# jungmannlab/picasso

Hardware: AMD Instinct MI355X
Metric: localizations/sec (7x7 ROI, MLE) (higher is better)
Workload: dtype f32+f64; 1 GPU; 10000-frame 512x512 uint16 simulated DNA-PAINT movie per GPU, 1001675 spots per GPU, 7x7 ROI MLE (sigmaxy), identify+cut+fit+table resident in HBM; frames=10000, height=512, width=512, box=7, max_it=100, localizations_total=1001675, mle_mode=refit, refit_spots_rank0=7346, frame_ranges_in_flight=2, all_gather=none

## Files before the change

__graft_entry__.py:

```python
from __future__ import annotations

import os
import subprocess
import sys

ROOT = os.path.dirname(os.path.abspath(__file__))
if ROOT not in sys.path:
    sys.path.insert(0, ROOT)


def build() -> None:
    csrc = os.path.join(ROOT, "picasso_amd", "csrc")
    jobs = str(min(4, os.cpu_count() or 1))
    subprocess.run(["make", "-C", csrc, "-j", jobs], check=True)
    subprocess.run(["make", "-C", os.path.join(ROOT, "oracle")], check=True)
    import picasso_amd
    from picasso_amd import _lib
    lib = _lib.load()
    assert lib.pmi_version() >= 100
    print(f"built {_lib.LIB_PATH} (ABI v{lib.pmi_version()}), {len(_lib.SYMBOLS)} symbols bound")


def smoke() -> None:
    import numpy as np
    import torch

    from oracle import oracle as orc
    from picasso_amd import _lib, backend, synth

    assert torch.cuda.is_available(), "smoke() needs a GPU"
    torch.cuda.set_device(0)
    _lib.require_gpu()
    cam = {"Baseline": 100.0, "Sensitivity": 1.0, "Gain": 1.0}
    movie = synth.simulate_movie(16, 256, 256, emitters_per_frame=40, seed=7, device="cuda:0")
    torch.cuda.synchronize()
    table = backend.localize_mle_device(movie.data_ptr(), np.uint16, tuple(movie.shape), 7, 5000, cam)
    host = movie.cpu().numpy()
    fr, y, x, ng = orc.identify(host, 5000, 7, threads=4)
    spots = orc.get_spots(host, fr, y, x, 7, cam)
    th, cr, ll, it = orc.gaussmle(spots, 1e-3, 100, "sigmaxy", threads=4)
    n = len(fr)
    assert n > 100 and len(table["frame"]) == n, (n, len(table["frame"]))
    assert np.array_equal(table["frame"], fr.astype(np.uint32))
    assert np.array_equal(table["net_gradient"], ng)
    assert np.array_equal(table["iterations"], it.astype(np.uint32)), int((table["iterations"] != it).sum())
    assert np.abs(table["x"] - (th[:, 0] + x - 3)).max() < 1e-3
    assert np.abs(table["y"] - (th[:, 1] + y - 3)).max() < 1e-3
# ... 11 lines not shown
```

picasso_amd/csrc/fit_common.h:

```cpp
#pragma once
#include <math.h>

#include "pmi_common.h"

namespace pmi {

#ifndef FIT_WAVES_N
#define FIT_WAVES_N 4
#endif
constexpr int FIT_WAVES = FIT_WAVES_N;
constexpr int FIT_NT = FIT_WAVES * PMI_WAVE;
constexpr int FIT_MAXPIX = PMI_MAX_BOX * PMI_MAX_BOX;

struct ConstDiv { float g, r; int fast; };
inline ConstDiv make_const_div(float g)
{
    ConstDiv c;
    c.g = g;
    c.r = (float)(1.0 / (double)g);
    c.fast = (g == g) && fabsf(g) > 1e-15f && fabsf(g) < 1e15f;
    if (g == 1.0f) c.fast = 2;
    return c;
}
__device__ __forceinline__ float div_const(float x, const ConstDiv &c)
// ... 27 lines not shown
#pragma unroll
        for (int i = 0; i < B; i++) v[i] = v[i] / c.g;
    }
}

struct FitParams {
    const float *spots;
    float *spots_out;
    const void *movie;
    const int32_t *frame, *y, *x;
    int dtype;
    int64_t Y, X;
    float baseline, sensitivity, gain;
    ConstDiv gdiv;
    int64_t N;
    const int64_t *d_n;
    int box;
    int libm_glibc;
    double eps;
    int max_it;
    float *thetas, *crlbs, *loglik;
    int32_t *iterations;
    unsigned long long *queue;
    unsigned *strict_queue;
    int64_t first;
    double *fisher;
    float eps_lo, eps_hi;
    int32_t *flag_list;
    unsigned *flag_count;
    unsigned *flag_reasons;
    const int32_t *final_list;
    const unsigned *final_list_n;
    unsigned char *refit_mark;
    float *ng_io;
    unsigned char *accept;
    int crop_y0, crop_x0, crop_cy, crop_cx;
    double min_ng;
    const int32_t *alist;
    const unsigned *alist_n;
    int32_t *alist_out;
    unsigned *alist_blk_out;
};
enum : unsigned { FLAG_MARGIN = 1u, FLAG_CURVATURE = 2u, FLAG_NARROW = 4u, FLAG_SWING = 8u, FLAG_WILD = 16u, FLAG_SLOW = 32u, FLAG_UNSTABLE = 64u };
constexpr int FLAG_REASONS = 7;
constexpr double FIT_UNSTABLE_LMAX = 1.9;
constexpr int FISHER_STRIDE = 21;
enum { FIT_STAGE_NEWTON = 1, FIT_STAGE_FINAL = 2, FIT_STAGE_INIT_ONLY = 4, FIT_STAGE_ITERATE_ONLY = 8 };
constexpr int FIT_SLOW_ITERATIONS = 64;
#ifndef PMI_MARGIN_GROWTH
#define PMI_MARGIN_GROWTH 0.0625f
#endif
constexpr float FIT_MARGIN_GROWTH = PMI_MARGIN_GROWTH;
constexpr float FIT_NARROW_SIGMA = 0.5f;
constexpr float FIT_WOBBLE_RATIO = 0.9f;
constexpr float FIT_WOBBLE_FLOOR = 1.9073486e-6f;
constexpr int FIT_WOBBLE_RUN = 3;
constexpr int FIT_WOBBLE_LATE = 9;
constexpr float FIT_TOP_FLAG = 16.0f;

template <int CTRL, int ROW_MASK = 0xf>
__device__ __forceinline__ float dpp_f(float v)
{
    return __builtin_bit_cast(float, __builtin_amdgcn_update_dpp(0, __builtin_bit_cast(int, v), CTRL, ROW_MASK, 0xf, false));
}
__device__ __forceinline__ float wave_sum(float v)
{
    v += dpp_f<0xB1>(v);
    v += dpp_f<0x4E>(v);
    v += dpp_f<0x141>(v);
    v += dpp_f<0x140>(v);
    v += dpp_f<0x142, 0xA>(v);
    v += dpp_f<0x143, 0xC>(v);
    return __builtin_bit_cast(float, __builtin_amdgcn_readlane(__builtin_bit_cast(int, v), 63));
}
template <int CTRL, int ROW_MASK = 0xf>
// ... 73 lines not shown
```

picasso_amd/csrc/gaussmle.hip:

```cpp
#include <algorithm>
#include <cmath>
#include <cstdlib>
#include <cstring>
#include <vector>

#include "fit_common.h"

namespace pmi {

__device__ __forceinline__ unsigned borderline(float D, int kk, float eps_lo, float eps_hi)
{
    const float wide = fmaxf(1.0f, (float)(kk - 1) * FIT_MARGIN_GROWTH);
    const float epsf = 0.5f * (eps_lo + eps_hi), epsm = 0.5f * (eps_hi - eps_lo) * wide;
    return ((D >= epsf - epsm && D < epsf + epsm) ? FLAG_MARGIN : 0u) | (kk > FIT_SLOW_ITERATIONS ? FLAG_SLOW : 0u);
}
struct StepHistory { float prev, prev2, wprev; int run; };
__device__ __forceinline__ bool wobbles(float st, float value, int kk, StepHistory &h)
{
    const float w = kk >= 3 ? (st - 2.0f * h.prev) + h.prev2 : 0.0f;
    const bool wob = w * h.wprev < 0.0f && fabsf(w) > FIT_WOBBLE_RATIO * fabsf(h.wprev) && fabsf(w) > FIT_WOBBLE_FLOOR * fabsf(value);
    h.run = wob ? h.run + 1 : 0;
    h.wprev = w; h.prev2 = h.prev; h.prev = st;
    return h.run >= FIT_WOBBLE_RUN || (h.run >= 2 && kk >= FIT_WOBBLE_LATE);
}
// ... 271 lines not shown
    for (int i = 0; i < NP; i++) for (int j = 0; j < NP; j++) V[i * NP + j] = (i == j) ? 1.0 : 0.0;
    for (int sweep = 0; sweep < 60; sweep++) {
        double off = 0.0;
        for (int a = 0; a < NP; a++) for (int b = a + 1; b < NP; b++) off += A[a * NP + b] * A[a * NP + b];
        if (off == 0.0) break;
        for (int a = 0; a < NP; a++)
            for (int b = a + 1; b < NP; b++) {
                double apq = A[a * NP + b];
                if (apq == 0.0) continue;
                double tau = (A[b * NP + b] - A[a * NP + a]) / (2.0 * apq);
                double tt = (tau >= 0 ? 1.0 : -1.0) / (fabs(tau) + sqrt(1.0 + tau * tau));
                double c = 1.0 / sqrt(1.0 + tt * tt), s = tt * c;
                for (int k = 0; k < NP; k++) { double x = A[k * NP + a], y = A[k * NP + b]; A[k * NP + a] = c * x - s * y; A[k * NP + b] = s * x + c * y; }
                for (int k = 0; k < NP; k++) { double x = A[a * NP + k], y = A[b * NP + k]; A[a * NP + k] = c * x - s * y; A[b * NP + k] = s * x + c * y; }
                for (int k = 0; k < NP; k++) { double x = V[k * NP + a], y = V[k * NP + b]; V[k * NP + a] = c * x - s * y; V[k * NP + b] = s * x + c * y; }
            }
    }
    double smax = 0.0;
    for (int i = 0; i < NP; i++) smax = fmax(smax, fabs(A[i * NP + i]));
    const double cutoff = 1e-15 * smax;
    for (int i = 0; i < NP; i++) {
        double acc = 0.0;
        for (int k = 0; k < NP; k++) { double lam = A[k * NP + k]; if (fabs(lam) > cutoff) acc += V[i * NP + k] * V[i * NP + k] / lam; }
        diag[i] = acc;
    }
}

template <int NP>
__global__ __launch_bounds__(256) void crlb_kernel(const double *__restrict__ fisher, int64_t first, int64_t N,
                                                   const int64_t *__restrict__ d_n, float *__restrict__ crlbs,
                                                   const int32_t *__restrict__ list, const unsigned *__restrict__ list_n,
                                                   int32_t *__restrict__ unstable, unsigned *__restrict__ unstable_n,
                                                   unsigned *__restrict__ reasons, const unsigned char *__restrict__ refit_mark,
                                                   const unsigned char *__restrict__ accept)
{
    int64_t n = N;
    if (d_n) { int64_t dn = *d_n; n = dn < n ? dn : n; }
    int64_t t = (int64_t)blockIdx.x * blockDim.x + threadIdx.x;
    int64_t sidx = first + t;
    if (list) {
        if (t >= (int64_t)*list_n) return;
        sidx = (int64_t)list[t];
        t = sidx - first;
    } else if (sidx >= n) return;
    else if (accept && !accept[sidx]) return;
    const double *f = fisher + t * FISHER_STRIDE;
    double M[36];
    {
        int e = 0;
#pragma unroll
        for (int k = 0; k < NP; k++)
#pragma unroll
            for (int l = k; l < NP; l++) { const double v = f[e++]; M[k * NP + l] = v; M[l * NP + k] = v; }
    }
    if (unstable && !(refit_mark && refit_mark[t])) {
        double dinv[NP], v[NP], lam = 0.0;
        bool ok = true;
#pragma unroll
        for (int i = 0; i < NP; i++) { const double m = M[i * NP + i]; ok = ok && m > 0.0 && m < 1e300; dinv[i] = 1.0 / sqrt(m); v[i] = 1.0 + 0.125 * (double)i; }
        if (ok) {
            double C[NP * NP], C2[NP * NP], t8 = 0.0;
#pragma unroll
            for (int i = 0; i < NP; i++)
#pragma unroll
                for (int k = 0; k < NP; k++) C[i * NP + k] = M[i * NP + k] * dinv[i] * dinv[k];
#pragma unroll
            for (int i = 0; i < NP; i++)
#pragma unroll
                for (int k = i; k < NP; k++) {
                    double a = 0.0;
#pragma unroll
                    for (int q = 0; q < NP; q++) a += C[i * NP + q] * C[q * NP + k];
                    C2[i * NP + k] = a; C2[k * NP + i] = a;
                }
#pragma unroll
            for (int i = 0; i < NP; i++)
#pragma unroll
                for (int k = i; k < NP; k++) {
// ... 239 lines not shown
    int32_t *acc_list = unstable_list + per_batch;
    unsigned *acc_blk = reinterpret_cast<unsigned *>(acc_list + per_batch);
    unsigned char *refit_mark = reinterpret_cast<unsigned char *>(acc_blk + acc_blocks);
    unsigned long long *queues = (unsigned long long *)ptr;
    unsigned *flag_counts = (unsigned *)(queues + 3 * nb);
    unsigned *strict_queues = flag_counts + 2 * nb;
    void *sptr = nullptr;
    if ((rc = scratch(SCR_STATS, 64, &sptr)) != PMI_OK) return rc;
    unsigned *stats = (unsigned *)sptr;
    hipLaunchKernelGGL(zero_words_kernel, dim3(1), dim3(256), 0, s, (unsigned *)ptr, (int)(nb * 10), stats, 16);
    p.flag_reasons = stats + 1;
    p.fisher = (double *)fptr;
    const int libm = mle_libm_now();
    const bool libm_all = libm != PMI_LIBM_DEVICE;
    p.libm_glibc = libm == PMI_LIBM_GLIBC || (libm == PMI_LIBM_AUTO && p.box <= 5);
    static const char *menv = tuning_env("PMI_MLE_MARGIN");
    const double margin = menv ? atof(menv) : g_mle_margin;
    const double ulp = ldexp(1.0, (int)floor(log2(std::max(1.0, p.box / 2.0))) - 23);
    const double margin_abs = std::max(p.eps * margin, 4.0 * ulp);
    p.eps_lo = (float)(p.eps - margin_abs);
    p.eps_hi = (float)(p.eps + margin_abs);
    const int ppl = (p.box * p.box + 63) / 64;
    const int64_t Ntotal = p.N;
    ScopedKernelTimer tm(s, &g_last_times.fit_ms);
    static const bool force_wave_per_spot = tuning_env("PMI_FIT_WAVE_PER_SPOT") != nullptr;
    const bool g8 = !force_wave_per_spot && p.box <= 15;
    float *cut = nullptr;
    static const bool no_keep = tuning_env("PMI_MLE_NO_KEEP") != nullptr;
    if (g8 && from_movie && mode != PMI_MLE_STRICT && !no_keep) {
        void *cptr = nullptr;
        if ((rc = scratch(SCR_STAGE_C, per_batch * (size_t)(p.box * p.box) * sizeof(float), &cptr)) != PMI_OK) return rc;
        cut = (float *)cptr;
    }
    p.spots_out = nullptr;
    if (p.ng_io && !(g8 && from_movie && cut)) { set_error("deferred exact stage outside the row-per-lane fit"); return PMI_ERR_ARG; }
    for (int64_t bi = 0; bi < nb; bi++) {
        p.first = bi * BATCH;
        p.N = std::min<int64_t>(Ntotal, p.first + BATCH);
        p.flag_list = mode == PMI_MLE_REFIT ? flag_list : nullptr;
        p.flag_count = flag_counts + bi;
        p.strict_queue = strict_queues + bi;
        p.refit_mark = mode == PMI_MLE_REFIT ? refit_mark : nullptr;
        if (p.refit_mark && !g8) PMI_HIP(hipMemsetAsync(refit_mark, 0, (size_t)(p.N - p.first), s));
        const int64_t count = p.N - p.first;
        const int64_t blocks = std::min<int64_t>((count + FIT_WAVES - 1) / FIT_WAVES, (int64_t)g_cu_count * 8);
        const dim3 grid((unsigned)std::max<int64_t>(blocks, 1));
        auto wave_per_spot = [&](int stages) {
            p.queue = queues + 3 * bi + (stages == FIT_STAGE_FINAL ? (p.final_list ? 2 : 1) : 0);
            if (method == PMI_MLE_SIGMAXY) {
                if (from_movie) launch_fit_ppl<6, true>(ppl, grid, s, p, stages); else launch_fit_ppl<6, false>(ppl, grid, s, p, stages);
            } else {
                if (from_movie) launch_fit_ppl<5, true>(ppl, grid, s, p, stages); else launch_fit_ppl<5, false>(ppl, grid, s, p, stages);
            }
        };
        if (mode != PMI_MLE_STRICT && g8 && from_movie && cut) {
            FitParams pi = p;
            pi.spots_out = cut;
            launch_fit_g8(pi, method, true, g_cu_count, state, FIT_STAGE_INIT_ONLY, s);
            PMI_HIP(hipGetLastError());
            FitParams q = p;
            q.spots = cut - p.first * (int64_t)(p.box * p.box);
            if (p.ng_io) {
                int32_t *al = nb == 1 && p.alist_out ? p.alist_out : acc_list;
                unsigned *ab = nb == 1 && p.alist_out ? p.alist_blk_out : acc_blk;
                if ((rc = build_accept_list(p.accept, p.first, p.N, p.d_n, ab, al, s)) != PMI_OK) return rc;
                q.alist = al;
                q.alist_n = ab + (count + ACC_BLOCK - 1) / ACC_BLOCK;
            }
            launch_fit_g8(q, method, false, g_cu_count, state, FIT_STAGE_ITERATE_ONLY, s);
            PMI_HIP(hipGetLastError());
            if (mode == PMI_MLE_REFIT)
                launch_fit_strict(q, method, false, flag_list, q.flag_count, count, g_cu_count, s);
            PMI_HIP(hipGetLastError());
            launch_fit_g8(q, method, false, g_cu_count, state, FIT_STAGE_FINAL, s);
        } else {
        if (mode == PMI_MLE_STRICT) {
            FitParams ps = p;
            ps.libm_glibc = libm_all;
            launch_fit_strict(ps, method, from_movie, nullptr, nullptr, count, g_cu_count, s);
        } else {
            if (g8) launch_fit_g8(p, method, from_movie, g_cu_count, state, FIT_STAGE_NEWTON, s);
            else wave_per_spot(FIT_STAGE_NEWTON);
            PMI_HIP(hipGetLastError());
            if (mode == PMI_MLE_REFIT)
                launch_fit_strict(p, method, from_movie, flag_list, p.flag_count, count, g_cu_count, s);
        }
        PMI_HIP(hipGetLastError());
        if (g8) launch_fit_g8(p, method, from_movie, g_cu_count, state, FIT_STAGE_FINAL, s);
        else wave_per_spot(FIT_STAGE_FINAL);
        }
        PMI_HIP(hipGetLastError());
        const unsigned cb = (unsigned)((count + 255) / 256);
        unsigned *unstable_n = flag_counts + nb + bi;
        auto crlb = [&](const int32_t *list, const unsigned *list_n, int32_t *out, unsigned *out_n) {
            if (method == PMI_MLE_SIGMAXY)
                hipLaunchKernelGGL((crlb_kernel<6>), dim3(cb), dim3(256), 0, s, p.fisher, p.first, p.N, p.d_n, p.crlbs, list, list_n, out, out_n, p.flag_reasons, p.refit_mark, p.accept);
            else
                hipLaunchKernelGGL((crlb_kernel<5>), dim3(cb), dim3(256), 0, s, p.fisher, p.first, p.N, p.d_n, p.crlbs, list, list_n, out, out_n, p.flag_reasons, p.refit_mark, p.accept);
        };
        const bool second = mode == PMI_MLE_REFIT;
        crlb(nullptr, nullptr, second ? unstable_list : nullptr, second ? unstable_n : nullptr);
        PMI_HIP(hipGetLastError());
        if (second) {
            FitParams r = p;
            r.strict_queue = strict_queues + nb + bi;
            if (cut) { r.spots = cut - p.first * (int64_t)(p.box * p.box); }
            const bool r_movie = cut ? false : from_movie;
            launch_fit_strict(r, method, r_movie, unstable_list, unstable_n, count, g_cu_count, s);
            PMI_HIP(hipGetLastError());
            r.final_list = unstable_list; r.final_list_n = unstable_n;
            if (g8) launch_fit_g8(r, method, r_movie, g_cu_count, state, FIT_STAGE_FINAL, s);
            else {
                FitParams keep = p;
                p = r;
                wave_per_spot(FIT_STAGE_FINAL);
                p = keep;
            }
            PMI_HIP(hipGetLastError());
            crlb(unstable_list, unstable_n, nullptr, nullptr);
            PMI_HIP(hipGetLastError());
        }
    }
    hipLaunchKernelGGL(flag_stats_kernel, dim3(1), dim3(1), 0, s, flag_counts, mode == PMI_MLE_REFIT ? 2 * nb : 0, stats);
    PMI_HIP(hipGetLastError());
    if ((rc = g_mle_stats.record(0, range, stats, s)) != PMI_OK) return rc;
    tm.stop();
    return PMI_OK;
}

static int read_last_stats(unsigned (&h)[16], hipStream_t s)
{
    if (g_mle_stats.valid()) PMI_HIP(hipStreamSynchronize(s));
    return g_mle_stats.read(h);
}

__global__ void cut_spots_kernel(const void *__restrict__ movie, int dtype, int64_t Y, int64_t X,
                                 const int32_t *__restrict__ frame, const int32_t *__restrict__ y,
                                 const int32_t *__restrict__ x, int64_t N, const int64_t *__restrict__ d_n,
                                 int box, float baseline, float sensitivity, ConstDiv gdiv, float *__restrict__ spots)
{
    int64_t n = N;
    if (d_n) { int64_t dn = *d_n; n = dn < n ? dn : n; }
    const int npix = box * box, h = box / 2;
    int64_t total = n * npix;
    for (int64_t t = (int64_t)blockIdx.x * blockDim.x + threadIdx.x; t < total; t += (int64_t)gridDim.x * blockDim.x) {
        int64_t i = t / npix;
        int q = (int)(t - i * npix);
        int a = q / box, c = q - a * box;
        float raw = load_movie_px(movie, dtype, ((int64_t)frame[i] * Y + (y[i] - h + a)) * X + (x[i] - h + c));
        spots[t] = div_const((raw - baseline) * sensitivity, gdiv);
    }
}
// ... 315 lines not shown
```

picasso_amd/csrc/gaussmle_g8.hip:

```cpp
#include <algorithm>

#include "fit_common.h"
#include "ng_common.h"

namespace pmi {

__device__ __forceinline__ float sum8(float v)
{
    v += dpp_f<0xB1>(v);
    v += dpp_f<0x4E>(v);
    v += dpp_f<0x141>(v);
    return v;
}
__device__ __forceinline__ float min8(float v)
{
    v = fminf(v, dpp_f<0xB1>(v));
    v = fminf(v, dpp_f<0x4E>(v));
    v = fminf(v, dpp_f<0x141>(v));
    return v;
}
__device__ __forceinline__ double sum8_d(double v)
{
    v += dpp_d<0xB1>(v);
    v += dpp_d<0x4E>(v);
// ... 516 lines not shown
    photons = (photons != photons) ? photons : (photons > 1.0 ? photons : 1.0);
    double a_sdy = 0.0, a_sy = 0.0, a_sdx = 0.0, a_sx = 0.0;
    if (rowok) {
        const float vm = d[H] - bg0;
        a_sdy = (double)vm * (double)((j - H) * (j - H));
        a_sy = (double)vm;
        if (j == H) {
#pragma unroll
            for (int i = 0; i < B; i++) {
                const float v2 = d[i] - bg0;
                a_sdx += (double)v2 * (double)((i - H) * (i - H));
                a_sx += (double)v2;
            }
        }
    }
    a_sdy = gsum_d<GS>(a_sdy); a_sy = gsum_d<GS>(a_sy); a_sdx = gsum_d<GS>(a_sdx); a_sx = gsum_d<GS>(a_sx);
    double isy = sqrt(a_sdy / a_sy), isx = sqrt(a_sdx / a_sx);
    if (!isfinite(isy)) isy = 0.01;
    if (!isfinite(isx)) isx = 0.01;
    if (isx == 0) isx = 0.01;
    if (isy == 0) isy = 0.01;

    float th[6], ms[6];
    th[0] = (float)com_x; th[1] = (float)com_y; th[2] = (float)photons; th[3] = bg0;
    if (NP == 6) { th[4] = (float)isx; th[5] = (float)isy; }
    else { th[4] = (float)((isx + isy) / 2); th[5] = 0.f; }
    ms[0] = th[4]; ms[1] = th[4];
    ms[2] = (float)(0.1 * (double)th[2]); ms[3] = (float)(0.1 * (double)th[3]);
    ms[4] = (float)(0.2 * (double)th[4]); ms[5] = (float)(0.2 * (double)th[5]);
    if (spot_ok && j == 0) {
        if (p.refit_mark) p.refit_mark[sidx - p.first] = 0;
        float4 *so = reinterpret_cast<float4 *>(state + (sidx - p.first) * 12);
        so[0] = make_float4(th[0], th[1], th[2], th[3]);
        so[1] = make_float4(th[4], th[5], ms[0], ms[1]);
        so[2] = make_float4(ms[2], ms[3], ms[4], ms[5]);
    }
}

template <int NP, int B, bool FROM_MOVIE>
__global__ __launch_bounds__(FIT_NT) void g8_iterate_kernel(FitParams p, const float *__restrict__ state)
{
    constexpr int GS = GroupOf<B>::GS, NSPW = 64 / GS;
    constexpr int REFILL_K = GS == 8 ? G8_REFILL_K : 1;
    __shared__ __attribute__((aligned(16))) float s_x[FIT_WAVES][NSPW][GLds<GS>::N];
    const int lane = threadIdx.x & 63, wid = threadIdx.x >> 6;
    const int g = lane / GS, j = lane & (GS - 1);
    const bool rowok = j < B;
    int64_t n = p.N;
    if (p.d_n) { int64_t dn = *p.d_n; n = dn < n ? dn : n; }
    const int64_t count = p.alist ? (int64_t)*p.alist_n : n - p.first;
    if (count <= 0) return;
    const int64_t total_waves = (int64_t)gridDim.x * FIT_WAVES;
    const int64_t chunk = (count + total_waves - 1) / total_waves;
    const int64_t wv = (int64_t)blockIdx.x * FIT_WAVES + __builtin_amdgcn_readfirstlane(wid);
    const int64_t base = p.alist ? 0 : p.first, lim = base + count;
    int64_t next = base + wv * chunk;
    const int64_t end = next + chunk < lim ? next + chunk : lim;
    if (next >= end) return;

    float *xs = &s_x[wid][g][0];
    float d[B], th[6], ms[6];
#pragma unroll
    for (int i = 0; i < B; i++) d[i] = 1.f;
#pragma unroll
    for (int l = 0; l < 6; l++) { th[l] = 1.f; ms[l] = 1.f; }
    LaneRole role = make_role<NP, B>(th, ms, j);
    int kk = 0;
    int64_t sidx = -1;
    bool active = false;
    unsigned flags = 0u;
    const unsigned long long below = (1ull << (lane & ~(GS - 1))) - 1ull;

    for (;;) {
        const unsigned long long pend = __ballot(!active && sidx >= 0 && j == 0);
        const unsigned long long empty = __ballot(!active && sidx < 0 && j == 0);
        const bool any_active = __any(active);
        if (__popcll(pend) >= REFILL_K || (pend != 0 && !any_active) || (empty != 0 && next < end)) {
            const unsigned gflag = gor_u<GS>(flags);
            if (!active && sidx >= 0 && j == 0) {
                float *to = p.thetas + sidx * 6;
#pragma unroll
                for (int l = 0; l < 5; l++) to[l] = th[l];
                to[5] = NP == 6 ? th[5] : th[4];
                p.iterations[sidx] = kk;
                if (gflag && p.flag_list) {
                    p.flag_list[atomicAdd(p.flag_count, 1u)] = (int32_t)sidx;
                    count_flag_reasons(p.flag_reasons, gflag);
                }
            }
            const unsigned long long want = pend | empty;
            const int64_t cand = next + __popcll(want & below);
            if (!active) {
                sidx = -1;
                if (cand < end) {
                    sidx = p.alist ? (int64_t)p.alist[cand] : cand;
                    const float4 *si = reinterpret_cast<const float4 *>(state + (sidx - p.first) * 12);
                    const float4 s0 = si[0], s1 = si[1], s2 = si[2];
                    th[0] = s0.x; th[1] = s0.y; th[2] = s0.z; th[3] = s0.w; th[4] = s1.x; th[5] = s1.y;
                    ms[0] = s1.z; ms[1] = s1.w; ms[2] = s2.x; ms[3] = s2.y; ms[4] = s2.z; ms[5] = s2.w;
                    load_row<B, FROM_MOVIE>(p, sidx, j, rowok, d);
                    role = make_role<NP, B>(th, ms, j);
                    kk = 0;
                    flags = 0u;
                    active = p.max_it > 0;
                    if (!active && j == 0) {
                        float *to = p.thetas + sidx * 6;
#pragma unroll
                        for (int l = 0; l < 5; l++) to[l] = th[l];
                        to[5] = NP == 6 ? th[5] : th[4];
                        p.iterations[sidx] = 0;
                        sidx = -1;
                    }
                }
            }
            next += __popcll(want);
            if (!__any(active)) {
                if (next >= end) break;
                continue;
            }
        } else if (!any_active) {
            break;
        }
        active = newton_step<NP, B>(d, th, role, xs, j, rowok, active, kk, p.eps, p.max_it, p.eps_lo, p.eps_hi, flags);
    }
}

template <int NP, int B, bool FROM_MOVIE>
__global__ __launch_bounds__(FIT_NT) void g8_final_kernel(FitParams p)
{
    constexpr int GS = GroupOf<B>::GS, NSPW = 64 / GS;
    __shared__ __attribute__((aligned(16))) double s_x[FIT_WAVES][NSPW][GS * 7];
    const int lane = threadIdx.x & 63, wid = threadIdx.x >> 6;
    const int g = lane / GS, j = lane & (GS - 1);
    const bool rowok = j < B;
    const float jf = (float)j;
    int64_t n = p.N;
    if (p.d_n) { int64_t dn = *p.d_n; n = dn < n ? dn : n; }
    int64_t sidx = p.first + ((int64_t)blockIdx.x * FIT_WAVES + wid) * NSPW + g;
    bool spot_ok = sidx < n;
    if (p.final_list) {
        const int64_t w0 = ((int64_t)blockIdx.x * FIT_WAVES + wid) * NSPW, items = (int64_t)*p.final_list_n;
        if (__builtin_amdgcn_readfirstlane((int)(w0 >= items))) return;
        spot_ok = w0 + g < items;
        sidx = spot_ok ? (int64_t)p.final_list[w0 + g] : p.first;
    } else if (__builtin_amdgcn_readfirstlane((int)(p.first + ((int64_t)blockIdx.x * FIT_WAVES + wid) * NSPW >= n))) return;
    else if (p.accept) spot_ok = spot_ok && p.accept[sidx] != 0;

    float d[B], th[6];
    load_row<B, FROM_MOVIE>(p, sidx, j, spot_ok && rowok, d);
#pragma unroll
    for (int l = 0; l < 6; l++) th[l] = spot_ok ? p.thetas[sidx * 6 + l] : 1.f;
    double *red = &s_x[wid][g][0];
    float *cols = reinterpret_cast<float *>(red);
    const float sgy = NP == 6 ? th[5] : th[4];
    const BTerms tx = boundary_terms(jf, th[0], th[4]);
    const BTerms ty = boundary_terms(jf, th[1], sgy);
    {
        float4 *c = reinterpret_cast<float4 *>(cols + j * 12);
        c[0] = make_float4(tx.A * tx.A, tx.A * tx.E, tx.A, tx.A * tx.S);
        c[1] = make_float4(tx.E * tx.E, tx.E, tx.E * tx.S, 1.0f);
        c[2] = make_float4(tx.S, tx.S * tx.S, 0.f, 0.f);
    }
    __builtin_amdgcn_wave_barrier();
    __threadfence_block();
    double T[10];
#pragma unroll
    for (int e = 0; e < 10; e++) T[e] = 0.0;
    float ll_loc = 0.f;
    const float N_ = th[2];
    const float NEy = N_ * ty.E;
#pragma unroll
    for (int i = 0; i < B; i++) {
        const float4 *c = reinterpret_cast<const float4 *>(cols + i * 12);
        const float4 c0 = c[0], c1 = c[1];
        const float2 c2 = *reinterpret_cast<const float2 *>(cols + i * 12 + 8);
        const float model = NEy * c1.y + th[3];
        if (rowok) {
            const double md = (double)model;
            double inv = (double)rcp_f32(model);
// ... 45 lines not shown
                const int e = j + GS * t - r0;
                if (e >= 0 && e < 7) {
                    double acc = 0.0;
#pragma unroll
                    for (int r = 0; r < B; r++) acc += red[r * 7 + e];
                    mine[t] = acc;
                }
            }
            __builtin_amdgcn_wave_barrier();
        }
    }
    double *fo = p.fisher + (sidx - p.first) * FISHER_STRIDE;
    if (spot_ok) {
#pragma unroll
        for (int t = 0; t < 3; t++)
            if (j + GS * t < NE_) fo[j + GS * t] = mine[t];
    }
    const float ll = gsum<GS>(ll_loc);
    if (spot_ok && j == 0) p.loglik[sidx] = ll;
}

template <int NP, int B, bool FROM_MOVIE>
static void launch_g8(const FitParams &p, float *state, int cu_count, int stages, hipStream_t s)
{
    constexpr int NSPW = 64 / GroupOf<B>::GS;
    const int64_t count = p.N - p.first;
    const int64_t waves = (count + NSPW - 1) / NSPW;
    const dim3 flat((unsigned)((waves + FIT_WAVES - 1) / FIT_WAVES));
    const int64_t pw = std::max<int64_t>(1, std::min<int64_t>((int64_t)cu_count * 24, (count + 63) / 64));
    const dim3 pers((unsigned)((pw + FIT_WAVES - 1) / FIT_WAVES));
    if (stages & (FIT_STAGE_NEWTON | FIT_STAGE_INIT_ONLY))
        hipLaunchKernelGGL((g8_init_kernel<NP, B, FROM_MOVIE>), flat, dim3(FIT_NT), 0, s, p, state);
    if (stages & (FIT_STAGE_NEWTON | FIT_STAGE_ITERATE_ONLY))
        hipLaunchKernelGGL((g8_iterate_kernel<NP, B, FROM_MOVIE>), pers, dim3(FIT_NT), 0, s, p, (const float *)state);
    if (stages & FIT_STAGE_FINAL)
        hipLaunchKernelGGL((g8_final_kernel<NP, B, FROM_MOVIE>), flat, dim3(FIT_NT), 0, s, p);
}

template <int NP, bool FROM_MOVIE>
static void launch_g8_box(const FitParams &p, float *state, int cu_count, int stages, hipStream_t s)
{
    switch (p.box) {
    case 3: launch_g8<NP, 3, FROM_MOVIE>(p, state, cu_count, stages, s); break;
    case 5: launch_g8<NP, 5, FROM_MOVIE>(p, state, cu_count, stages, s); break;
    case 7: launch_g8<NP, 7, FROM_MOVIE>(p, state, cu_count, stages, s); break;
    case 9: launch_g8<NP, 9, FROM_MOVIE>(p, state, cu_count, stages, s); break;
    case 11: launch_g8<NP, 11, FROM_MOVIE>(p, state, cu_count, stages, s); break;
    case 13: launch_g8<NP, 13, FROM_MOVIE>(p, state, cu_count, stages, s); break;
    default: launch_g8<NP, 15, FROM_MOVIE>(p, state, cu_count, stages, s); break;
    }
}

bool launch_fit_g8(const FitParams &p, int method, bool from_movie, int cu_count, float *state, int stages, hipStream_t s)
{
    if (p.box > 15) return false;
    if (method == PMI_MLE_SIGMAXY) {
        if (from_movie) launch_g8_box<6, true>(p, state, cu_count, stages, s); else launch_g8_box<6, false>(p, state, cu_count, stages, s);
    } else {
        if (from_movie) launch_g8_box<5, true>(p, state, cu_count, stages, s); else launch_g8_box<5, false>(p, state, cu_count, stages, s);
    }
    return true;
}

}
```

picasso_amd/csrc/pmi_common.h:

```cpp
#pragma once
#include <hip/hip_runtime.h>
#include <stdint.h>
#include <stdio.h>
#include <stdlib.h>
#include <string.h>

#include <functional>

#include "../../include/picasso_hip.h"

#define PMI_WAVE 64

namespace pmi {

#ifdef PMI_TUNING
inline const char *tuning_env(const char *name) { return getenv(name); }
#else
inline const char *tuning_env(const char *) { return nullptr; }
#endif

void set_error(const char *fmt, ...);
int hip_fail(hipError_t e, const char *what, const char *file, int line);

#define PMI_HIP(call)                                                          \
// ... 2 lines not shown
        if (e_ != hipSuccess) return pmi::hip_fail(e_, #call, __FILE__, __LINE__); \
    } while (0)

constexpr int PMI_MAX_DEVICES = 16;
int current_device();
int checked_device(int *device);
int device_cu_count();

enum ScratchSlot {
    SCR_RECORDS = 0,
    SCR_RECORDS2,
    SCR_FRAME_COUNT,
    SCR_COUNTERS,
    SCR_IDS,
    SCR_FIT,
    SCR_STAGE_A,
    SCR_STAGE_B,
    SCR_STAGE_C,
    SCR_STAGE_D,
    SCR_ROWS,
    SCR_NARROW,
    SCR_GATES,
    SCR_STATS,
    SCR_LQ_STATS,
    SCR_NUM
};
int scratch(int slot, size_t bytes, void **ptr);
int scratch_release_all();
int scratch_enter_inner();
void scratch_leave_inner(int was);
unsigned scratch_generation(int slot);
unsigned scratch_generation_of(int device, int user_bank, int slot);
int scratch_user_bank();
struct SideLane { hipStream_t s2 = nullptr; hipEvent_t ev_start = nullptr, ev_scan_a = nullptr, ev_b = nullptr, stats_done[2] = {nullptr, nullptr}; };
int side_lane(int pipeline, SideLane **lane);

struct LastFitStats {
    int device = 0, bank = 0, slot = 0;
    unsigned generation = 0;
    const unsigned *buf[2] = {nullptr, nullptr};
    hipEvent_t done[2] = {nullptr, nullptr};
    int record(int pipeline, int range, const unsigned *stats, hipStream_t s);
    bool valid() const;
    int read(unsigned (&h)[16]) const;
};

struct FusedRanges {
    size_t ids_bytes;
    int64_t capc;
    int64_t cap;
    bool rejects;
    std::function<int(void *ids, int64_t f_lo, int64_t f_hi, int64_t *d_cnt, hipStream_t st)> scan;
    std::function<int(void *ids, const int64_t *d_rows, int range, hipStream_t st)> fit;
    std::function<const unsigned *(void *ids)> accepted;
    std::function<int(void *ids, const int64_t *d_rows, const int64_t *d_row0, hipStream_t st)> table;
};
int fused_ranges(const FusedRanges &c, int pipeline, int64_t F, int64_t Y, int64_t X, int64_t f_lo, int64_t f_hi,
                 int64_t *d_out_n, hipStream_t s);

struct Record {
    int32_t frame;
    uint32_t yx;
    int32_t pad;
    float ng;
};
__host__ __device__ __forceinline__ uint32_t pack_yx(int y, int x) { return ((uint32_t)y << 16) | (uint32_t)(x & 0xffff); }
constexpr uint32_t NG_DEFERRED_BITS = 0x7fc0d1feu;
// ... 33 lines not shown
```

picasso_amd/csrc/runtime.hip:

```cpp
#include <stdarg.h>

#include <mutex>

#include "pmi_common.h"

namespace pmi {

static thread_local char g_err[512] = "";
bool g_kernel_timing = false;
KernelTimes g_last_times = {0.f, 0.f};
int g_localize_ranges = 2;
thread_local char g_last_scan_kernel[128] = "";

void set_error(const char *fmt, ...)
{
    va_list ap;
    va_start(ap, fmt);
    vsnprintf(g_err, sizeof(g_err), fmt, ap);
    va_end(ap);
}

int hip_fail(hipError_t e, const char *what, const char *file, int line)
{
    set_error("HIP error %d (%s) in %s at %s:%d", (int)e, hipGetErrorString(e), what, file, line);
// ... 77 lines not shown
        for (auto &bank : g_scratch_banks[dev])
            for (auto &b : bank)
                if (b.p) { if (hipFree(b.p) != hipSuccess) rc = PMI_ERR_HIP; b.p = nullptr; b.bytes = 0; }
    }
    (void)hipSetDevice(was);
    return rc;
}
int scratch_select_bank(int bank)
{
    if (bank < 0 || bank >= SCR_USER_BANKS) { set_error("scratch bank %d out of range", bank); return PMI_ERR_ARG; }
    g_scratch_bank = bank;
    return PMI_OK;
}
int scratch_enter_inner() { const int was = g_scratch_bank; g_scratch_bank = was % SCR_USER_BANKS + SCR_USER_BANKS; return was; }
void scratch_leave_inner(int was) { g_scratch_bank = was; }

static SideLane g_side_lanes[PMI_MAX_DEVICES][SCR_USER_BANKS][2];
static std::mutex g_side_mu;
int side_lane(int pipeline, SideLane **lane)
{
    int dev = 0;
    const int rc = checked_device(&dev);
    if (rc != PMI_OK) return rc;
    std::lock_guard<std::mutex> lk(g_side_mu);
    SideLane &sd = g_side_lanes[dev][scratch_user_bank()][pipeline ? 1 : 0];
    if (!sd.s2) {
        hipStream_t s2 = nullptr;
        PMI_HIP(hipStreamCreateWithFlags(&s2, hipStreamNonBlocking));
        PMI_HIP(hipEventCreateWithFlags(&sd.ev_start, hipEventDisableTiming));
        PMI_HIP(hipEventCreateWithFlags(&sd.ev_scan_a, hipEventDisableTiming));
        PMI_HIP(hipEventCreateWithFlags(&sd.ev_b, hipEventDisableTiming));
        PMI_HIP(hipEventCreateWithFlags(&sd.stats_done[0], hipEventDisableTiming));
        PMI_HIP(hipEventCreateWithFlags(&sd.stats_done[1], hipEventDisableTiming));
        sd.s2 = s2;
    }
    *lane = &sd;
    return PMI_OK;
}

int LastFitStats::record(int pipeline, int range, const unsigned *stats, hipStream_t s)
{
    SideLane *lane = nullptr;
    const int rc = side_lane(pipeline, &lane);
    if (rc != PMI_OK) return rc;
    PMI_HIP(hipEventRecord(lane->stats_done[range], s));
    if (range == 0) buf[1] = nullptr;
    buf[range] = stats;
    done[range] = lane->stats_done[range];
    slot = pipeline ? SCR_LQ_STATS : SCR_STATS;
    device = current_device();
    bank = scratch_user_bank();
    generation = scratch_generation_of(device, bank, slot);
    return PMI_OK;
}
bool LastFitStats::valid() const { return buf[0] && generation == scratch_generation_of(device, bank, slot); }
int LastFitStats::read(unsigned (&h)[16]) const
{
    for (unsigned &v : h) v = 0;
    if (!valid()) return PMI_OK;
    for (int k = 0; k < 2; k++) {
        if (!buf[k]) continue;
        unsigned part[16];
        PMI_HIP(hipEventSynchronize(done[k]));
        PMI_HIP(hipMemcpy(part, buf[k], 64, hipMemcpyDeviceToHost));
        for (int i = 0; i < 16; i++) h[i] += part[i];
    }
// ... 25 lines not shown
    const int64_t lo = f_lo < 0 ? 0 : f_lo, hi = f_hi > F - 1 ? F - 1 : f_hi, nf = hi - lo + 1;
    const bool two = g_localize_ranges == 2 && !g_kernel_timing && nf >= 16 && (double)nf * (double)Y * (double)X >= 2.5e8;
    void *ptr = nullptr, *cptr = nullptr;
    int rc;
    if ((rc = scratch(SCR_ROWS, 8 * sizeof(int64_t), &cptr)) != PMI_OK) return rc;
    int64_t *n = (int64_t *)cptr, *rows = n + 2;
    if ((rc = scratch(SCR_IDS, c.ids_bytes, &ptr)) != PMI_OK) return rc;
    void *ids[2] = {ptr, nullptr};
    auto table_rows = [&](hipStream_t st) {
        hipLaunchKernelGGL(table_rows_kernel, dim3(1), dim3(1), 0, st, (const int64_t *)n, c.rejects ? c.accepted(ids[0]) : nullptr,
                           (const int64_t *)(two ? n + 1 : nullptr), c.rejects && two ? c.accepted(ids[1]) : nullptr, c.capc,
                           c.cap, rows, d_out_n);
    };
    auto fit_rows = [&](int r, hipStream_t st) -> const int64_t * {
        if (!c.rejects && r == (two ? 1 : 0)) {
            table_rows(st);
            return rows + 2 + r;
        }
        hipLaunchKernelGGL(fit_rows_kernel, dim3(1), dim3(1), 0, st, (const int64_t *)(n + r), c.capc, rows + r);
        return rows + r;
    };
    if (!two) {
        if ((rc = c.scan(ids[0], f_lo, f_hi, n, s)) != PMI_OK) return rc;
        if ((rc = c.fit(ids[0], fit_rows(0, s), 0, s)) != PMI_OK) return rc;
    } else {
        SideLane *side_p = nullptr;
        if ((rc = side_lane(pipeline, &side_p)) != PMI_OK) return rc;
        SideLane &side = *side_p;
        const int64_t mid = lo + nf / 2 - 1;
        PMI_HIP(hipEventRecord(side.ev_start, s));
        PMI_HIP(hipStreamWaitEvent(side.s2, side.ev_start, 0));
        struct Join {
            SideLane &sd; hipStream_t st; bool done = false;
            ~Join() { if (!done) { (void)hipEventRecord(sd.ev_b, sd.s2); (void)hipStreamWaitEvent(st, sd.ev_b, 0); } }
        } join{side, s};
        if ((rc = c.scan(ids[0], lo, mid, n, s)) != PMI_OK) return rc;
        const int64_t *rows_a = fit_rows(0, s);
        PMI_HIP(hipEventRecord(side.ev_scan_a, s));
        if ((rc = c.fit(ids[0], rows_a, 0, s)) != PMI_OK) return rc;
        PMI_HIP(hipStreamWaitEvent(side.s2, side.ev_scan_a, 0));
        const int outer = scratch_enter_inner();
        rc = scratch(SCR_IDS, c.ids_bytes, &ids[1]);
        if (rc == PMI_OK) rc = c.scan(ids[1], mid + 1, hi, n + 1, side.s2);
        if (rc == PMI_OK) rc = c.fit(ids[1], fit_rows(1, side.s2), 1, side.s2);
        scratch_leave_inner(outer);
        if (rc != PMI_OK) return rc;
        PMI_HIP(hipEventRecord(side.ev_b, side.s2));
        PMI_HIP(hipStreamWaitEvent(s, side.ev_b, 0));
        join.done = true;
    }
    if (c.rejects) table_rows(s);
    if ((rc = c.table(ids[0], rows + 2, nullptr, s)) != PMI_OK) return rc;
    if (two && (rc = c.table(ids[1], rows + 3, rows + 4, s)) != PMI_OK) return rc;
    PMI_HIP(hipGetLastError());
    return PMI_OK;
}

void release_fft_plans();

}

extern "C" {

int pmi_version(void) { return 110; }

const char *pmi_last_error(void) { return pmi::g_err; }

// ... 90 lines not shown
```

Baseline: 368.0 million localizations/s.

## Fork MLE final/CRLB tail onto side stream, overlapping with strict refit

In refit mode the iterate kernel now writes its flag bits into an unused slot of the per-spot state. The final-stage and CRLB kernels for unflagged spots then run on a dedicated tail stream, skipping any spot marked in the state. Meanwhile the main stream runs the strict refit, then final and CRLB for only the flagged list, and the two streams join with events. The point is to overlap the long-tail strict refit with the bulk tail work, at the cost of extra streams, events and a repurposed state slot (ms[1] is now read back as ms[0]).

```diff
diff --git a/__graft_entry__.py b/__graft_entry__.py
--- a/__graft_entry__.py
+++ b/__graft_entry__.py
@@ -13,6 +13,7 @@
     csrc = os.path.join(ROOT, "picasso_amd", "csrc")
     jobs = str(min(4, os.cpu_count() or 1))
     subprocess.run(["make", "-C", csrc, "-j", jobs], check=True)
+    subprocess.run(["make", "-C", csrc, "-j", jobs, "tuning"], check=True)
     subprocess.run(["make", "-C", os.path.join(ROOT, "oracle")], check=True)
     import picasso_amd
     from picasso_amd import _lib
diff --git a/picasso_amd/csrc/fit_common.h b/picasso_amd/csrc/fit_common.h
--- a/picasso_amd/csrc/fit_common.h
+++ b/picasso_amd/csrc/fit_common.h
@@ -83,6 +83,7 @@
     const int32_t *final_list;
     const unsigned *final_list_n;
     unsigned char *refit_mark;
+    const float *skip_marked;
     float *ng_io;
     unsigned char *accept;
     int crop_y0, crop_x0, crop_cy, crop_cx;
@@ -92,6 +93,11 @@
     int32_t *alist_out;
     unsigned *alist_blk_out;
 };
+constexpr unsigned FIT_STATE_MARK = 7u;
+__device__ __forceinline__ unsigned newton_mark(const float *state, int64_t t)
+{
+    return reinterpret_cast<const unsigned *>(state)[(unsigned)t * 12u + FIT_STATE_MARK];
+}
 enum : unsigned { FLAG_MARGIN = 1u, FLAG_CURVATURE = 2u, FLAG_NARROW = 4u, FLAG_SWING = 8u, FLAG_WILD = 16u, FLAG_SLOW = 32u, FLAG_UNSTABLE = 64u };
 constexpr int FLAG_REASONS = 7;
 constexpr double FIT_UNSTABLE_LMAX = 1.9;
diff --git a/picasso_amd/csrc/gaussmle.hip b/picasso_amd/csrc/gaussmle.hip
--- a/picasso_amd/csrc/gaussmle.hip
+++ b/picasso_amd/csrc/gaussmle.hip
@@ -327,7 +327,7 @@
                                                    const int32_t *__restrict__ list, const unsigned *__restrict__ list_n,
                                                    int32_t *__restrict__ unstable, unsigned *__restrict__ unstable_n,
                                                    unsigned *__restrict__ reasons, const unsigned char *__restrict__ refit_mark,
-                                                   const unsigned char *__restrict__ accept)
+                                                   const unsigned char *__restrict__ accept, const float *__restrict__ skip_marked)
 {
     int64_t n = N;
     if (d_n) { int64_t dn = *d_n; n = dn < n ? dn : n; }
@@ -339,6 +339,7 @@
         t = sidx - first;
     } else if (sidx >= n) return;
     else if (accept && !accept[sidx]) return;
+    else if (skip_marked && newton_mark(skip_marked, t)) return;
     const double *f = fisher + t * FISHER_STRIDE;
     double M[36];
     {
@@ -644,6 +645,16 @@
         if ((rc = scratch(SCR_STAGE_C, per_batch * (size_t)(p.box * p.box) * sizeof(float), &cptr)) != PMI_OK) return rc;
         cut = (float *)cptr;
     }
+    static const bool tail_serial = tuning_env("PMI_MLE_TAIL_SERIAL") != nullptr;
+    const bool fork = mode == PMI_MLE_REFIT && g8 && !tail_serial;
+    SideLane *lane = nullptr;
+    if (fork && (rc = side_lane(0, &lane)) != PMI_OK) return rc;
+    const hipStream_t ts = fork ? lane->tail[range] : nullptr;
+    struct TailJoin {
+        SideLane *sd; const int r; const hipStream_t ts, st; bool open = false;
+        int join() { open = false; PMI_HIP(hipEventRecord(sd->ev_tail[r], ts)); PMI_HIP(hipStreamWaitEvent(st, sd->ev_tail[r], 0)); return PMI_OK; }
+        ~TailJoin() { if (open) (void)join(); }
+    } tail{lane, range, ts, s};
     p.spots_out = nullptr;
     if (p.ng_io && !(g8 && from_movie && cut)) { set_error("deferred exact stage outside the row-per-lane fit"); return PMI_ERR_ARG; }
     for (int64_t bi = 0; bi < nb; bi++) {
@@ -665,53 +676,64 @@
                 if (from_movie) launch_fit_ppl<5, true>(ppl, grid, s, p, stages); else launch_fit_ppl<5, false>(ppl, grid, s, p, stages);
             }
         };
+        FitParams f = p;
+        bool f_movie = from_movie;
         if (mode != PMI_MLE_STRICT && g8 && from_movie && cut) {
             FitParams pi = p;
             pi.spots_out = cut;
             launch_fit_g8(pi, method, true, g_cu_count, state, FIT_STAGE_INIT_ONLY, s);
             PMI_HIP(hipGetLastError());
-            FitParams q = p;
-            q.spots = cut - p.first * (int64_t)(p.box * p.box);
+            f.spots = cut - p.first * (int64_t)(p.box * p.box);
+            f_movie = false;
             if (p.ng_io) {
                 int32_t *al = nb == 1 && p.alist_out ? p.alist_out : acc_list;
                 unsigned *ab = nb == 1 && p.alist_out ? p.alist_blk_out : acc_blk;
                 if ((rc = build_accept_list(p.accept, p.first, p.N, p.d_n, ab, al, s)) != PMI_OK) return rc;
-                q.alist = al;
-                q.alist_n = ab + (count + ACC_BLOCK - 1) / ACC_BLOCK;
-            }
-            launch_fit_g8(q, method, false, g_cu_count, state, FIT_STAGE_ITERATE_ONLY, s);
-            PMI_HIP(hipGetLastError());
-            if (mode == PMI_MLE_REFIT)
-                launch_fit_strict(q, method, false, flag_list, q.flag_count, count, g_cu_count, s);
-            PMI_HIP(hipGetLastError());
-            launch_fit_g8(q, method, false, g_cu_count, state, FIT_STAGE_FINAL, s);
-        } else {
-        if (mode == PMI_MLE_STRICT) {
+                f.alist = al;
+                f.alist_n = ab + (count + ACC_BLOCK - 1) / ACC_BLOCK;
+            }
+            launch_fit_g8(f, method, false, g_cu_count, state, FIT_STAGE_ITERATE_ONLY, s);
+        } else if (mode == PMI_MLE_STRICT) {
             FitParams ps = p;
             ps.libm_glibc = libm_all;
             launch_fit_strict(ps, method, from_movie, nullptr, nullptr, count, g_cu_count, s);
         } else {
             if (g8) launch_fit_g8(p, method, from_movie, g_cu_count, state, FIT_STAGE_NEWTON, s);
             else wave_per_spot(FIT_STAGE_NEWTON);
-            PMI_HIP(hipGetLastError());
-            if (mode == PMI_MLE_REFIT)
-                launch_fit_strict(p, method, from_movie, flag_list, p.flag_count, count, g_cu_count, s);
-        }
-        PMI_HIP(hipGetLastError());
-        if (g8) launch_fit_g8(p, method, from_movie, g_cu_count, state, FIT_STAGE_FINAL, s);
-        else wave_per_spot(FIT_STAGE_FINAL);
         }
         PMI_HIP(hipGetLastError());
         const unsigned cb = (unsigned)((count + 255) / 256);
         unsigned *unstable_n = flag_counts + nb + bi;
-        auto crlb = [&](const int32_t *list, const unsigned *list_n, int32_t *out, unsigned *out_n) {
+        auto crlb = [&](hipStream_t st, const int32_t *list, const unsigned *list_n, int32_t *out, unsigned *out_n, const unsigned char *mark, const float *skip) {
             if (method == PMI_MLE_SIGMAXY)
-                hipLaunchKernelGGL((crlb_kernel<6>), dim3(cb), dim3(256), 0, s, p.fisher, p.first, p.N, p.d_n, p.crlbs, list, list_n, out, out_n, p.flag_reasons, p.refit_mark, p.accept);
+                hipLaunchKernelGGL((crlb_kernel<6>), dim3(cb), dim3(256), 0, st, p.fisher, p.first, p.N, p.d_n, p.crlbs, list, list_n, out, out_n, p.flag_reasons, mark, p.accept, skip);
             else
-                hipLaunchKernelGGL((crlb_kernel<5>), dim3(cb), dim3(256), 0, s, p.fisher, p.first, p.N, p.d_n, p.crlbs, list, list_n, out, out_n, p.flag_reasons, p.refit_mark, p.accept);
+                hipLaunchKernelGGL((crlb_kernel<5>), dim3(cb), dim3(256), 0, st, p.fisher, p.first, p.N, p.d_n, p.crlbs, list, list_n, out, out_n, p.flag_reasons, mark, p.accept, skip);
         };
         const bool second = mode == PMI_MLE_REFIT;
-        crlb(nullptr, nullptr, second ? unstable_list : nullptr, second ? unstable_n : nullptr);
+        if (fork) {
+            PMI_HIP(hipEventRecord(lane->ev_fork[range], s));
+            PMI_HIP(hipStreamWaitEvent(ts, lane->ev_fork[range], 0));
+            tail.open = true;
+            FitParams t = f;
+            t.skip_marked = state;
+            launch_fit_g8(t, method, f_movie, g_cu_count, state, FIT_STAGE_FINAL, ts);
+            crlb(ts, nullptr, nullptr, unstable_list, unstable_n, nullptr, state);
+            launch_fit_strict(f, method, f_movie, flag_list, f.flag_count, count, g_cu_count, s);
+            FitParams l = f;
+            l.final_list = flag_list; l.final_list_n = f.flag_count;
+            launch_fit_g8(l, method, f_movie, g_cu_count, state, FIT_STAGE_FINAL, s);
+            crlb(s, flag_list, f.flag_count, nullptr, nullptr, nullptr, nullptr);
+            PMI_HIP(hipGetLastError());
+            if ((rc = tail.join()) != PMI_OK) return rc;
+        } else {
+            if (mode == PMI_MLE_REFIT) launch_fit_strict(f, method, f_movie, flag_list, f.flag_count, count, g_cu_count, s);
+            PMI_HIP(hipGetLastError());
+            if (g8) launch_fit_g8(f, method, f_movie, g_cu_count, state, FIT_STAGE_FINAL, s);
+            else wave_per_spot(FIT_STAGE_FINAL);
+            PMI_HIP(hipGetLastError());
+            crlb(s, nullptr, nullptr, second ? unstable_list : nullptr, second ? unstable_n : nullptr, p.refit_mark, nullptr);
+        }
         PMI_HIP(hipGetLastError());
         if (second) {
             FitParams r = p;
@@ -729,7 +751,7 @@
                 p = keep;
             }
             PMI_HIP(hipGetLastError());
-            crlb(unstable_list, unstable_n, nullptr, nullptr);
+            crlb(s, unstable_list, unstable_n, nullptr, nullptr, nullptr, nullptr);
             PMI_HIP(hipGetLastError());
         }
     }
diff --git a/picasso_amd/csrc/gaussmle_g8.hip b/picasso_amd/csrc/gaussmle_g8.hip
--- a/picasso_amd/csrc/gaussmle_g8.hip
+++ b/picasso_amd/csrc/gaussmle_g8.hip
@@ -572,13 +572,13 @@
         if (p.refit_mark) p.refit_mark[sidx - p.first] = 0;
         float4 *so = reinterpret_cast<float4 *>(state + (sidx - p.first) * 12);
         so[0] = make_float4(th[0], th[1], th[2], th[3]);
-        so[1] = make_float4(th[4], th[5], ms[0], ms[1]);
+        so[1] = make_float4(th[4], th[5], ms[0], 0.f);
         so[2] = make_float4(ms[2], ms[3], ms[4], ms[5]);
     }
 }
 
 template <int NP, int B, bool FROM_MOVIE>
-__global__ __launch_bounds__(FIT_NT) void g8_iterate_kernel(FitParams p, const float *__restrict__ state)
+__global__ __launch_bounds__(FIT_NT) void g8_iterate_kernel(FitParams p, float *state)
 {
     constexpr int GS = GroupOf<B>::GS, NSPW = 64 / GS;
     constexpr int REFILL_K = GS == 8 ? G8_REFILL_K : 1;
@@ -624,6 +624,7 @@
                 to[5] = NP == 6 ? th[5] : th[4];
                 p.iterations[sidx] = kk;
                 if (gflag && p.flag_list) {
+                    reinterpret_cast<unsigned *>(state)[(unsigned)(sidx - p.first) * 12u + FIT_STATE_MARK] = gflag;
                     p.flag_list[atomicAdd(p.flag_count, 1u)] = (int32_t)sidx;
                     count_flag_reasons(p.flag_reasons, gflag);
                 }
@@ -637,7 +638,7 @@
                     const float4 *si = reinterpret_cast<const float4 *>(state + (sidx - p.first) * 12);
                     const float4 s0 = si[0], s1 = si[1], s2 = si[2];
                     th[0] = s0.x; th[1] = s0.y; th[2] = s0.z; th[3] = s0.w; th[4] = s1.x; th[5] = s1.y;
-                    ms[0] = s1.z; ms[1] = s1.w; ms[2] = s2.x; ms[3] = s2.y; ms[4] = s2.z; ms[5] = s2.w;
+                    ms[0] = s1.z; ms[1] = s1.z; ms[2] = s2.x; ms[3] = s2.y; ms[4] = s2.z; ms[5] = s2.w;
                     load_row<B, FROM_MOVIE>(p, sidx, j, rowok, d);
                     role = make_role<NP, B>(th, ms, j);
                     kk = 0;
@@ -684,7 +685,10 @@
         spot_ok = w0 + g < items;
         sidx = spot_ok ? (int64_t)p.final_list[w0 + g] : p.first;
     } else if (__builtin_amdgcn_readfirstlane((int)(p.first + ((int64_t)blockIdx.x * FIT_WAVES + wid) * NSPW >= n))) return;
-    else if (p.accept) spot_ok = spot_ok && p.accept[sidx] != 0;
+    else {
+        if (p.accept) spot_ok = spot_ok && p.accept[sidx] != 0;
+        if (p.skip_marked && spot_ok) spot_ok = newton_mark(p.skip_marked, sidx - p.first) == 0u;
+    }
 
     float d[B], th[6];
     load_row<B, FROM_MOVIE>(p, sidx, j, spot_ok && rowok, d);
@@ -796,7 +800,7 @@
     if (stages & (FIT_STAGE_NEWTON | FIT_STAGE_INIT_ONLY))
         hipLaunchKernelGGL((g8_init_kernel<NP, B, FROM_MOVIE>), flat, dim3(FIT_NT), 0, s, p, state);
     if (stages & (FIT_STAGE_NEWTON | FIT_STAGE_ITERATE_ONLY))
-        hipLaunchKernelGGL((g8_iterate_kernel<NP, B, FROM_MOVIE>), pers, dim3(FIT_NT), 0, s, p, (const float *)state);
+        hipLaunchKernelGGL((g8_iterate_kernel<NP, B, FROM_MOVIE>), pers, dim3(FIT_NT), 0, s, p, state);
     if (stages & FIT_STAGE_FINAL)
         hipLaunchKernelGGL((g8_final_kernel<NP, B, FROM_MOVIE>), flat, dim3(FIT_NT), 0, s, p);
 }
diff --git a/picasso_amd/csrc/pmi_common.h b/picasso_amd/csrc/pmi_common.h
--- a/picasso_amd/csrc/pmi_common.h
+++ b/picasso_amd/csrc/pmi_common.h
@@ -58,7 +58,12 @@
 unsigned scratch_generation(int slot);
 unsigned scratch_generation_of(int device, int user_bank, int slot);
 int scratch_user_bank();
-struct SideLane { hipStream_t s2 = nullptr; hipEvent_t ev_start = nullptr, ev_scan_a = nullptr, ev_b = nullptr, stats_done[2] = {nullptr, nullptr}; };
+struct SideLane {
+    hipStream_t s2 = nullptr;
+    hipEvent_t ev_start = nullptr, ev_scan_a = nullptr, ev_b = nullptr, stats_done[2] = {nullptr, nullptr};
+    hipStream_t tail[2] = {nullptr, nullptr};
+    hipEvent_t ev_fork[2] = {nullptr, nullptr}, ev_tail[2] = {nullptr, nullptr};
+};
 int side_lane(int pipeline, SideLane **lane);
 
 struct LastFitStats {
diff --git a/picasso_amd/csrc/runtime.hip b/picasso_amd/csrc/runtime.hip
--- a/picasso_amd/csrc/runtime.hip
+++ b/picasso_amd/csrc/runtime.hip
@@ -133,6 +133,11 @@
         PMI_HIP(hipEventCreateWithFlags(&sd.ev_b, hipEventDisableTiming));
         PMI_HIP(hipEventCreateWithFlags(&sd.stats_done[0], hipEventDisableTiming));
         PMI_HIP(hipEventCreateWithFlags(&sd.stats_done[1], hipEventDisableTiming));
+        for (int r = 0; r < 2; r++) {
+            PMI_HIP(hipStreamCreateWithFlags(&sd.tail[r], hipStreamNonBlocking));
+            PMI_HIP(hipEventCreateWithFlags(&sd.ev_fork[r], hipEventDisableTiming));
+            PMI_HIP(hipEventCreateWithFlags(&sd.ev_tail[r], hipEventDisableTiming));
+        }
         sd.s2 = s2;
     }
     *lane = &sd;
@@ -224,7 +229,11 @@
         PMI_HIP(hipStreamWaitEvent(side.s2, side.ev_start, 0));
         struct Join {
             SideLane &sd; hipStream_t st; bool done = false;
-            ~Join() { if (!done) { (void)hipEventRecord(sd.ev_b, sd.s2); (void)hipStreamWaitEvent(st, sd.ev_b, 0); } }
+            ~Join() {
+                if (done) return;
+                for (int r = 0; r < 2; r++) { (void)hipEventRecord(sd.ev_tail[r], sd.tail[r]); (void)hipStreamWaitEvent(st, sd.ev_tail[r], 0); }
+                (void)hipEventRecord(sd.ev_b, sd.s2); (void)hipStreamWaitEvent(st, sd.ev_b, 0);
+            }
         } join{side, s};
         if ((rc = c.scan(ids[0], lo, mid, n, s)) != PMI_OK) return rc;
         const int64_t *rows_a = fit_rows(0, s);
```

Result: no change. 367.8 million localizations/s (-0.1%).
